# kevinh-e/BetaOne

Hardware: AMD Instinct MI355X
Metric: mcts_nodes_per_sec (higher is better)
Workload: dtype f32 (3 x f16 split, f32 accumulate)

## Files before the change

betaone_amd/csrc/bo_engine.cpp:

```cpp
#include "../../include/betaone_engine.h"
#include "../../include/betaone_lab.h"

#include "bo_tree.h"
#include "bo_fastw.h"
#include "bo_info.h"
#include "bo_select_wide.h"
#include "bo_replay.h"
#include "bo_train.h"
#include "bo_metrics.h"
#include "bo_pgn.h"
#include "bo_san.h"
#include "bo_analyse.h"
#include "bo_reanalyse.h"
#include "bo_perft.h"
#include "bo_mate.h"
#include "bo_anchor.h"
#include "bo_book.h"
#include "bo_merge.h"
#include "bo_tb.h"
#include "bo_nn_fused.h"
#include "bo_conv.h"
#include "bo_tower.h"
#include "bo_tower_wg.h"
#include "bo_tower_h.h"
#include "bo_tower_s.h"
#include "bo_tower_s16.h"
#include "bo_tower_h16.h"
#include "bo_heads.h"
#include "bo_tower_b1.h"
#include "bo_rt.h"
#include "bo_hostrng.h"

#include <math.h>
#include <stdio.h>
#include <string.h>
#include <string>
#include <vector>
#include <algorithm>
#include <deque>
#include <memory>
#include <type_traits>

static thread_local std::string g_err;
static int fail(int code, const std::string &msg) {
    g_err = msg;
    return code;
}
#define RT(call)                                                                                     \
    do {                                                                                             \
        int _rc = (call);                                                                            \
        if (_rc != 0) return fail(BO_E_HIP, std::string(#call) + ": " + rt_errstr(_rc));             \
    } while (0)

struct bo_engine {
    Eng d;
    FastW f;
    int fast_reuse = 1;
    int sel_profile = 0, sel_pending = 0;
    long long sel_launches = 0;
    double sel_ms = 0.0;
#if !defined(BO_WAVE_EMU)
// ... 482 lines not shown

static int step_launch(bo_engine *e, const float *policy_dev, const float *value_dev, int policy_kind, float *nn_in_dev, void *stream, const StepTail &vt) {
    e->prefetch_valid = false;
    if (e->fast) {
        const int rows = e->d.c.G * e->f.L;
        if (policy_kind != BO_POLICY_NONE) RT(RT_LAUNCH(bo_k_fw_apply, rows, stream, e->d, e->f, policy_dev, value_dev, policy_kind));
#if !defined(BO_WAVE_EMU)
        if (e->sel_profile) {
            if (!e->sel_ev0) { RT((int)hipEventCreate(&e->sel_ev0)); RT((int)hipEventCreate(&e->sel_ev1)); }
            if (e->sel_pending) {
                float ms = 0.0f;
                RT((int)hipEventSynchronize(e->sel_ev1));
                RT((int)hipEventElapsedTime(&ms, e->sel_ev0, e->sel_ev1));
                e->sel_ms += ms; e->sel_launches++; e->sel_pending = 0;
            }
            RT((int)hipEventRecord(e->sel_ev0, (hipStream_t)stream));
        }
#endif
        RT(launch_fw_select(e, policy_kind != BO_POLICY_NONE ? e->f.row_val : value_dev, policy_kind, stream));
#if !defined(BO_WAVE_EMU)
        if (e->sel_profile) { RT((int)hipEventRecord(e->sel_ev1, (hipStream_t)stream)); e->sel_pending = 1; }
#endif
        RT(RT_LAUNCH(bo_k_fw_leaf, rows, stream, e->d, e->f, nn_in_dev));
    } else {
        if (e->d.tb_n > 0 && (e->d.tb_flags & TBF_SEARCH)) RT(RT_LAUNCH(bo_k_step_tb, e->d.c.G, stream, e->d, policy_dev, value_dev, policy_kind, nn_in_dev, vt));
        else RT(RT_LAUNCH(bo_k_step, e->d.c.G, stream, e->d, policy_dev, value_dev, policy_kind, nn_in_dev, vt));
    }
    return BO_OK;
}
extern "C" int bo_step(bo_engine *e, const float *policy_dev, const float *value_dev, int policy_kind, float *nn_in_dev,
                       void *stream) {
    if (!e || !nn_in_dev) return fail(BO_E_ARG, "null argument");
    if (policy_kind != BO_POLICY_NONE && (!policy_dev || !value_dev)) return fail(BO_E_ARG, "policy/value required");
    return step_launch(e, policy_dev, value_dev, policy_kind, nn_in_dev, stream, StepTail{nullptr, nullptr, nullptr, nullptr, 0});
}
extern "C" int bo_step_heads(bo_engine *e, const float *logits_dev, const float *vpart_dev, const float *b1_dev, const float *w2_dev,
                             const float *b2_dev, int rows, float *nn_in_dev, void *stream) {
    if (!e || !nn_in_dev || !logits_dev || !vpart_dev || !b1_dev || !w2_dev || !b2_dev) return fail(BO_E_ARG, "null argument");
    if (e->fast) return fail(BO_E_CONFIG, "bo_step_heads: the reference-semantics search only (fast mode evaluates rows, not games)");
    if (rows < e->d.c.G) return fail(BO_E_ARG, "bo_step_heads: the partial sums must hold a row per game (rows >= G)");
    return step_launch(e, logits_dev, nullptr, BO_POLICY_LOGITS, nn_in_dev, stream, StepTail{vpart_dev, b1_dev, w2_dev, b2_dev, rows});
}

extern "C" int bo_search_poll(bo_engine *e, int32_t *n_running, int32_t *n_requested, int32_t *requested_mask, void *stream) {
    if (!e) return fail(BO_E_ARG, "null engine");
    const size_t G = (size_t)e->d.c.G;
    RT(rt_d2h(e->h_info, e->d_info_blk, 2 * G * 4, stream));
    const int *ph = e->h_info, *rq = e->h_info + G;
    RT(rt_sync(stream));
    int run = 0, req = 0;
    for (size_t g = 0; g < G; g++) {
        bool r = ph[g] == PH_RUN;
        bool q = r && rq[g] >= 0;
        run += r; req += q;
        if (requested_mask) requested_mask[g] = q ? 1 : 0;
    }
    if (n_running) *n_running = run;
    if (n_requested) *n_requested = req;
    return BO_OK;
}

extern "C" int bo_search_stop(bo_engine *e, const int32_t *stop_mask, int32_t *sims_done, void *stream) {
    if (!e) return fail(BO_E_ARG, "null engine");
    const size_t G = (size_t)e->d.c.G;
    const int *d_mask = nullptr;
    if (stop_mask) {
        memcpy(e->h_go, stop_mask, G * 4);
        RT(rt_h2d(e->d_go, e->h_go, G * 4, stream));
        d_mask = e->d_go;
    }
    if (e->fast) {
        e->prefetch_valid = false;
        RT(RT_LAUNCH(bo_k_fw_stop, e->d.c.G, stream, e->d, e->f, d_mask));
    } else {
// ... 3329 lines not shown
```

betaone_amd/csrc/bo_heads.h:

```cpp
#pragma once
#if !defined(BO_WAVE_EMU)
#include <hip/hip_runtime.h>
#include "bo_tower.h"

#define BO_HEADS_NA 4672
#define BO_HEADS_KP 128
#define BO_HEADS_KV 2048
#define BO_HEADS_NH 256
#define BO_HEADS_KS 16
#define BO_HEADS_PITCH 132

struct bo_heads_args {
    const void *p, *v;
    const float *wp, *bp, *w1, *b1, *w2, *b2;
    float *policy_out, *value_out;
    float *vpart;
    int B, softmax;
    int pb;
};
static inline int bo_heads_policy_boards(int batch) { return batch > 64 ? 128 : batch > 32 ? 64 : 32; }

struct bo_heads_pair {
    const int32_t *sel = nullptr;
    const float *wp = nullptr, *bp = nullptr, *w1 = nullptr, *b1 = nullptr, *w2 = nullptr, *b2 = nullptr;
// ... 107 lines not shown
            const int hb = 32 * (wave & 1), bb = 32 * (wave >> 1);
            bo_f32x4 acc[2][2];
#pragma unroll
            for (int c = 0; c < 2; c++)
#pragma unroll
                for (int rt = 0; rt < 2; rt++) acc[c][rt] = bo_f32x4{0, 0, 0, 0};
#pragma unroll
            for (int t = 0; t < BO_HEADS_KV / BO_HEADS_KS / 16; t++) {
                bo_f32x4 fw[2], fv[2];
#pragma unroll
                for (int c = 0; c < 2; c++) fw[c] = *reinterpret_cast<const bo_f32x4 *>(&tileW[(hb + 16 * c + i) * BO_HEADS_PITCH + 16 * t + 4 * kq]);
#pragma unroll
                for (int rt = 0; rt < 2; rt++) fv[rt] = *reinterpret_cast<const bo_f32x4 *>(&tileA[(bb + 16 * rt + i) * BO_HEADS_PITCH + 16 * t + 4 * kq]);
#pragma unroll
                for (int e = 0; e < 4; e++)
#pragma unroll
                    for (int c = 0; c < 2; c++)
#pragma unroll
                        for (int rt = 0; rt < 2; rt++) acc[c][rt] = __builtin_amdgcn_mfma_f32_16x16x4f32(fw[c][e], fv[rt][e], acc[c][rt], 0, 0, 0);
            }
#pragma unroll
            for (int c = 0; c < 2; c++)
#pragma unroll
                for (int rt = 0; rt < 2; rt++) {
                    const int row = r0 + bb + 16 * rt + i;
                    if (row < B && (only_net < 0 || (pr.sel[row] != 0) == only_net))
                        *reinterpret_cast<bo_f32x4 *>(a.vpart + ((size_t)ks * B + row) * BO_HEADS_NH + h0 + hb + 16 * c + 4 * kq) = acc[c][rt];
                }
        }
    }
}

template <bool PAIR>
__device__ __forceinline__ void bo_heads_rows_body(const bo_heads_args &a, const bo_heads_pair &q) {
    __shared__ float sred[8];
    const int tid = threadIdx.x, lane = tid & 63, wave = __builtin_amdgcn_readfirstlane(tid >> 6);
    const int B = a.B, row = (int)blockIdx.x;
    const float *b1 = a.b1, *w2 = a.w2, *b2 = a.b2;
    if constexpr (PAIR) {
        if (__builtin_amdgcn_readfirstlane(q.sel[row]) != 0) { b1 = q.b1; w2 = q.w2; b2 = q.b2; }
    }
    float part[BO_HEADS_KS];
#pragma unroll
    for (int ks = 0; ks < BO_HEADS_KS; ks++) part[ks] = a.vpart[((size_t)ks * B + row) * BO_HEADS_NH + tid];
    bo_f32x4 *r4 = reinterpret_cast<bo_f32x4 *>(a.policy_out + (size_t)row * BO_HEADS_NA);
    constexpr int N4 = BO_HEADS_NA / 4, IT = (N4 + 255) / 256;
    const float ninf = -__builtin_inff();
    bo_f32x4 x[IT];
    float mx = ninf;
    if (a.softmax) {
#pragma unroll
        for (int u = 0; u < IT; u++) {
            const int k = tid + 256 * u;
            x[u] = k < N4 ? r4[k] : bo_f32x4{ninf, ninf, ninf, ninf};
        }
    }
    float hsum = 0.0f;
#pragma unroll
    for (int ks = 0; ks < BO_HEADS_KS; ks++) hsum += part[ks];
    hsum += b1[tid];
    hsum = (hsum > 0.0f ? hsum : 0.0f) * w2[tid];
    if (a.softmax) {
#pragma unroll
        for (int u = 0; u < IT; u++) mx = fmaxf(mx, fmaxf(fmaxf(x[u][0], x[u][1]), fmaxf(x[u][2], x[u][3])));
    }
#pragma unroll
    for (int m = 32; m >= 1; m >>= 1) { mx = fmaxf(mx, __shfl_xor(mx, m, 64)); hsum += __shfl_xor(hsum, m, 64); }
    if (lane == 0) { sred[wave] = mx; sred[4 + wave] = hsum; }
    __syncthreads();
    mx = fmaxf(fmaxf(sred[0], sred[1]), fmaxf(sred[2], sred[3]));
    if (tid == 0) a.value_out[row] = tanhf(((sred[4] + sred[5]) + (sred[6] + sred[7])) + b2[0]);
    if (a.softmax) {
        float sum = 0.0f;
#pragma unroll
        for (int u = 0; u < IT; u++) {
            if (tid + 256 * u < N4) {
#pragma unroll
                for (int e = 0; e < 4; e++) { x[u][e] = expf(x[u][e] - mx); sum += x[u][e]; }
            }
        }
#pragma unroll
        for (int m = 32; m >= 1; m >>= 1) sum += __shfl_xor(sum, m, 64);
        __syncthreads();
        if (lane == 0) sred[wave] = sum;
        __syncthreads();
        sum = (sred[0] + sred[1]) + (sred[2] + sred[3]);
#pragma unroll
        for (int u = 0; u < IT; u++) {
            const int k = tid + 256 * u;
            if (k < N4) r4[k] = bo_f32x4{x[u][0] / sum, x[u][1] / sum, x[u][2] / sum, x[u][3] / sum};
        }
    }
}

extern "C" __global__ void __launch_bounds__(256)
bo_k_heads_rows(bo_heads_args a) { bo_heads_rows_body<false>(a, bo_heads_pair{}); }

extern "C" __global__ void __launch_bounds__(256)
bo_k_heads_rows_pair(bo_heads_args a, bo_heads_pair q) { bo_heads_rows_body<true>(a, q); }

typedef _Float16 bo_hh8 __attribute__((ext_vector_type(8)));

#ifndef BO_HEADS_NT_STORES
#define BO_HEADS_NT_STORES 1
// ... 224 lines not shown
```

betaone_amd/csrc/bo_tree.h:

```cpp
#pragma once
#include "bo_chess.h"
#include "bo_tb_probe.h"
#include <math.h>

#define BO_CH_CAP 32
#define BO_PATH_CAP 1024
#define BO_RES_CAP 256
#define BO_PLANES 120
#ifndef BO_PROF_SLOTS
#define BO_PROF_SLOTS 16
#endif
#define BO_ROW (BO_PLANES * 64)

enum { PH_IDLE = 0, PH_RUN = 1, PH_DONE = 2 };
enum { ST_OK = 0, ST_NODE_OVERFLOW = 1, ST_DEPTH_OVERFLOW = 2, ST_NAN_SCORE = 4, ST_PLY_OVERFLOW = 8,
       ST_ILLEGAL_ACTION = 16, ST_UL_OVERFLOW = 32, ST_TRK_OVERFLOW = 64 };
enum { POLICY_NONE = 0, POLICY_LOGITS = 1, POLICY_PROBS = 2 };

struct EngCfg {
    int G, S, B;
    int NCAP, PLY_CAP, TRK_CAP;
    int nstride;
    int UL_MAX, CH_MAX;
    float cpuct, keep;
// ... 692 lines not shown
            const float a = e.c.keep * sh.probs[idx];
            const double s2 = (double)a + e.c.eps * nz[j];
            sh.probs[idx] = (float)s2;
        }
        bo_sync();
        const float sum = np_sum_4672(sh.probs);
        const float denom = sum + 1e-12f;
        for (int j = lane; j < n; j += 64) sh.pv[j] = finite_or_zero(sh.probs[move_to_index(mv[j])] / denom, &bad);
        bo_sync();
    }
    if (bo_ballot(bad) != 0) *flags |= ST_NAN_SCORE;
    for (int j = lane; j < n; j += 64) {
        int r = stable_rank(sh.pv, n, j);
        if (r < m) sh.rank_of[BO_CH_CAP + r] = j;
    }
    bo_sync();
    for (int r = 0; r < m; r++) {
        const int j = sh.rank_of[BO_CH_CAP + r];
        bool present = false;
        for (int k = 0; k < m; k++) present = present || sh.rank_of[k] == j;
        if (!present) {
            if (lane == 0) {
                init_node(e, no, 1 + nch, 0, sh.pv[j], mv[j], make_move(P, mv[j]));
                e.root_child_rank[(size_t)g * 2 * BO_CH_CAP + nch] = j;
            }
            nch++;
        }
    }
    if (lane == 0) { e.first_child[no] = 1; e.n_children[no] = nch; e.root_nch[g] = nch; }
    *n_nodes_io = 1 + nch;
    bo_sync();
}

struct StepTail { const float *vpart, *b1, *w2, *b2; int rows; };
struct TailRegs { float part[4][16], b1[4], w2[4], b2; };
BO_DEV void tail_load(const StepTail &t, int g, TailRegs &r) {
    const int lane = bo_lane();
    BO_UNROLL
    for (int w = 0; w < 4; w++) {
        BO_UNROLL
        for (int ks = 0; ks < 16; ks++) r.part[w][ks] = t.vpart[((size_t)ks * t.rows + g) * 256 + lane + 64 * w];
        r.b1[w] = t.b1[lane + 64 * w];
        r.w2[w] = t.w2[lane + 64 * w];
    }
    r.b2 = t.b2[0];
}
BO_DEV float tail_value(const TailRegs &r) {
    float s[4];
    BO_UNROLL
    for (int w = 0; w < 4; w++) {
        float h = 0.0f;
        BO_UNROLL
        for (int ks = 0; ks < 16; ks++) h += r.part[w][ks];
        h += r.b1[w];
        s[w] = (h > 0.0f ? h : 0.0f) * r.w2[w];
    }
    for (int m = 32; m >= 1; m >>= 1) {
        BO_UNROLL
        for (int w = 0; w < 4; w++) s[w] = s[w] + bo_shfl_xor_f(s[w], m);
    }
    return tanhf(((s[0] + s[1]) + (s[2] + s[3])) + r.b2);
}

BO_DEV void apply_leaf(const Eng &e, int g, int leaf, const float *row, int kind, const float *value_of, const StepTail &vt, StepShared &sh,
                       int *n_ul_io, int *flags) {
    const size_t no = NOFF(e, g);
    const int lane = bo_lane();
    const int n = e.req_nlegal[g];
    const bo_mv *mv = e.req_moves + (size_t)g * BO_MAX_MOVES;
    int slot = *n_ul_io;
    if (slot >= e.c.UL_MAX) { *flags |= ST_UL_OVERFLOW; slot = e.c.UL_MAX - 1; }
    const size_t uo = (size_t)g * e.c.UL_MAX + slot;
    float value;
    bool bad = false;
    if (kind == POLICY_PROBS) {
        value = value_of[g];
        for (int j = lane; j < n; j += 64) sh.pv[j] = finite_or_zero(row[move_to_index(mv[j])], &bad);
    } else {
        float mx, sum;
        if (vt.vpart) {
            TailRegs tr;
            tail_load(vt, g, tr);
            row_max_sum(row, &mx, &sum);
            value = tail_value(tr);
        } else {
            value = value_of[g];
            row_max_sum(row, &mx, &sum);
        }
        for (int j = lane; j < n; j += 64) sh.pv[j] = finite_or_zero(bo_exp_row(row[move_to_index(mv[j])] - mx) / sum, &bad);
    }
    bo_sync();
    value = finite_or_zero(value, &bad);
    if (bo_ballot(bad) != 0) *flags |= ST_NAN_SCORE;
    const int M = n < e.c.CH_MAX ? n : e.c.CH_MAX;
    for (int j = lane; j < n; j += 64) {
        int r = stable_rank(sh.pv, n, j);
        if (r < M) { e.ul_move[uo * BO_CH_CAP + r] = mv[j]; e.ul_prior[uo * BO_CH_CAP + r] = sh.pv[j]; }
    }
    if (lane == 0) {
        e.ul_node[uo] = leaf;
        e.ul_nlegal[uo] = n;
        e.ul_value[uo] = value;
        e.eval_slot[no + leaf] = (short)slot;
    }
    *n_ul_io = slot + 1;
    bo_sync();
}


// ... 534 lines not shown
```

betaone_amd/engine.py:

```python
from __future__ import annotations

import ctypes as C
import os
from typing import Dict, List, Optional, Sequence, Tuple

import numpy as np
import torch

NUM_ACTIONS = 4672
INPUT_CHANNELS = 120
ROW_FLOATS = 120 * 64
MAX_LEGAL = 256
RES_CAP = 256
POLICY_NONE, POLICY_LOGITS, POLICY_PROBS = 0, 1, 2

STATUS_BITS = {1: "node overflow", 2: "depth overflow", 4: "NaN or infinite evaluation (prior or value)", 8: "ply overflow",
               16: "illegal action", 32: "leaf cache overflow", 64: "tracker overflow", 128: "position range outside the array",
               256: "pi wider than the record's rows"}
ST_PLY_OVERFLOW, ST_ILLEGAL_ACTION = 8, 16
ST_PI_OVERFLOW = 256
ST_NODE_OVERFLOW = 1
ST_DEPTH_OVERFLOW = 2
ST_NAN_SCORE = 4

# ... 46 lines not shown
                             ("pi_n", "<i4"), ("played_prob", "<f4"), ("has_old", "<i4"), ("agree", "<i4"), ("tv", "<f4"), ("phase", "<i4"),
                             ("status", "<i4"), ("ply", "<i4"), ("sims_done", "<i4"), ("watch", "<i4"), ("reserved", "<i4")])
PH_IDLE, PH_RUN, PH_DONE = 0, 1, 2
INFO_LINES, INFO_PV = 8, 24
INFO_LINE_DTYPE = np.dtype([("move", "<i4"), ("visits", "<i4"), ("w", "<f4"), ("prior", "<f4"), ("pv_len", "<i4"), ("pv", "<i4", (INFO_PV,)),
                            ("reserved", "<i4", (3,))])
INFO_DTYPE = np.dtype([("phase", "<i4"), ("status", "<i4"), ("terminal", "<i4"), ("n_legal", "<i4"), ("sims_done", "<i4"),
                       ("root_visits", "<i4"), ("arena_top", "<i4"), ("arena_granules", "<i4"), ("watch", "<i4"), ("n_lines", "<i4"),
                       ("reserved", "<i4", (6,)), ("line", INFO_LINE_DTYPE, (INFO_LINES,))])
INFO_WORDS = INFO_DTYPE.itemsize // 4


class BoHeadWeights(C.Structure):
    _fields_ = [("wp", C.c_void_p), ("bp", C.c_void_p), ("w1", C.c_void_p), ("b1", C.c_void_p), ("w2", C.c_void_p), ("b2", C.c_void_p)]


_I32P = C.POINTER(C.c_int32)
_F32P = C.POINTER(C.c_float)
_F64P = C.POINTER(C.c_double)
_TRAIN_BATCH = [C.c_int32, C.c_int32, C.c_void_p, C.c_int32, C.c_void_p, C.c_int32] + [C.c_void_p] * 3

_SYMBOLS = {
    "bo_abi_version": (C.c_int, []),
    "bo_last_error": (C.c_char_p, []),
    "bo_engine_create": (C.c_int, [C.POINTER(BoConfig), C.c_int, C.POINTER(C.c_void_p)]),
    "bo_engine_destroy": (None, [C.c_void_p]),
    "bo_games_reset": (C.c_int, [C.c_void_p, C.c_int, _I32P, C.POINTER(C.c_char_p), C.POINTER(C.c_char_p), C.c_void_p]),
    "bo_games_reset_ex": (C.c_int, [C.c_void_p, C.c_int, _I32P, C.POINTER(C.c_char_p), C.POINTER(C.c_char_p),
                                    C.POINTER(BoPosition), _I32P, C.POINTER(BoPosition), _I32P, _I32P, C.c_void_p]),
    "bo_root_info": (C.c_int, [C.c_void_p, _I32P, _I32P, _I32P, C.c_void_p]),
    "bo_search_begin": (C.c_int, [C.c_void_p, _I32P, _F64P, C.c_void_p, C.c_void_p]),
    "bo_step": (C.c_int, [C.c_void_p, C.c_void_p, C.c_void_p, C.c_int, C.c_void_p, C.c_void_p]),
    "bo_step_heads": (C.c_int, [C.c_void_p] * 6 + [C.c_int, C.c_void_p, C.c_void_p]),
    "bo_search_poll": (C.c_int, [C.c_void_p, _I32P, _I32P, _I32P, C.c_void_p]),
    "bo_search_stop": (C.c_int, [C.c_void_p, _I32P, _I32P, C.c_void_p]),
    "bo_search_close": (C.c_int, [C.c_void_p, C.c_void_p]),
    "bo_search_info": (C.c_int, [C.c_void_p, C.c_int32, C.c_void_p, C.c_void_p]),
    "bo_search_result": (C.c_int, [C.c_void_p, _I32P, _I32P, _F32P, _I32P, _I32P, _I32P, C.c_void_p]),
    "bo_play": (C.c_int, [C.c_void_p, _I32P, C.c_void_p]),
    "bo_game_export": (C.c_int, [C.c_void_p, C.c_int, C.POINTER(BoPosition), _I32P, C.c_int32, _I32P, C.c_void_p]),
    "bo_game_encode": (C.c_int, [C.c_void_p, C.c_int, C.c_int, C.c_int, C.c_void_p, C.c_void_p]),
    "bo_rng_seed": (C.c_int, [C.c_void_p, C.c_int, C.c_uint32]),
    "bo_rng_state": (C.c_int, [C.c_void_p, C.c_int, C.c_int, C.POINTER(C.c_uint32), _I32P, _I32P, _F64P]),
    "bo_selfplay_sample": (C.c_int, [C.c_void_p, _I32P, _I32P, C.c_int32, C.c_double, C.c_double, _I32P, _I32P, _F32P,
                                     _I32P, _I32P, C.c_void_p]),
    "bo_selfplay_turn": (C.c_int, [C.c_void_p, _I32P, _I32P, C.c_int32, C.c_double, C.c_double, _I32P, _I32P, _F32P, _I32P, _I32P, _I32P,
                                   C.c_void_p, _I32P, _I32P, _I32P, C.c_int32, _I32P, C.c_void_p]),
    "bo_selfplay_noise": (C.c_int, [C.c_void_p, C.c_void_p]),
    "bo_selfplay_autoturn": (C.c_int, [C.c_void_p, _I32P, _I32P, C.c_int32, C.c_double, C.c_double, _I32P, C.c_void_p, C.c_int32, C.c_void_p]),
    "bo_selfplay_autoturn_ready": (C.c_int, [C.c_void_p, _I32P]),
    "bo_selfplay_autoturn_collect": (C.c_int, [C.c_void_p, _I32P, _I32P, _F32P, _I32P, _I32P, _I32P, _I32P, _I32P, _I32P]),
    "bo_selfplay_autoturn_collect_ex": (C.c_int, [C.c_void_p, _I32P, _I32P, _F32P, _I32P, _I32P, _I32P, _I32P, _I32P, _F32P, _I32P, _I32P]),
    "bo_engine_root_values": (C.c_int, [C.c_void_p, C.c_int32]),
    "bo_selfplay_resign": (C.c_int, [C.c_void_p, _I32P, C.c_float, C.c_int32]),
    "bo_search_root_value": (C.c_int, [C.c_void_p, _F32P, C.c_void_p]),
    "bo_pgn_movetext_text": (C.c_int, [C.c_int32, C.c_void_p, C.c_void_p, C.c_int32, C.c_int32, C.c_char_p, _I32P, C.c_char_p, C.c_char_p,
                                       C.c_char_p, C.c_int64, C.POINTER(C.c_int64)]),
    "bo_search_result_prefetch": (C.c_int, [C.c_void_p, C.c_void_p]),
    "bo_selfplay_begun": (C.c_int, [C.c_void_p, _I32P, _I32P, _I32P]),
    "bo_selfplay_begin": (C.c_int, [C.c_void_p, _I32P, C.c_void_p, _I32P, _I32P, _I32P, C.c_void_p]),
    "bo_records_encode": (C.c_int, [C.c_int, C.POINTER(BoPosition), C.c_int, C.c_int, C.c_void_p, C.c_void_p]),
    "bo_fast_options": (C.c_int, [C.c_void_p, C.c_int32, C.c_int32, C.c_int32]),
    "bo_nn_tower_status": (C.c_int, [C.c_void_p, _I32P, C.c_void_p]),
    "bo_nn_tower_word": (C.c_int, [C.c_void_p, C.POINTER(C.c_void_p)]),
    "bo_replay_create": (C.c_int, [C.c_int64, C.c_int, C.c_int, C.POINTER(C.c_void_p)]),
    "bo_replay_add_game": (C.c_int, [C.c_void_p, C.c_int32, C.POINTER(BoPosition), C.c_int32, _I32P, _I32P, _F32P, _F32P, C.POINTER(C.c_int64), C.c_void_p]),
# ... 90 lines not shown
    "bo_anchor": (C.c_int, [C.c_int, C.c_int32, C.POINTER(C.c_char_p), C.c_void_p, C.c_int32, C.c_int64, C.c_uint32, C.c_void_p, C.c_void_p,
                            C.c_void_p, C.POINTER(C.c_int64), C.c_void_p]),
    "bo_anchor_eval": (C.c_int, [C.c_int, C.c_int32, C.c_void_p, C.c_void_p, C.c_void_p]),
    "bo_anchor_q": (C.c_int, [C.c_int, C.c_int32, C.POINTER(C.c_char_p), C.c_void_p, C.c_int32, C.c_int32, C.c_int64, C.c_uint32, C.c_void_p,
                              C.c_void_p, C.c_void_p, C.POINTER(C.c_int64), C.c_void_p]),
}
_LAB_SYMBOLS = {
    "bo_debug_tree": (C.c_int, [C.c_void_p, C.c_int, C.POINTER(BoNode), C.c_int32, _I32P, C.c_void_p]),
    "bo_debug_search_state": (C.c_int, [C.c_void_p, _I32P, C.c_void_p]),
    "bo_debug_fast": (C.c_int, [C.c_void_p, C.c_int, _I32P, C.c_int32, _I32P, C.c_void_p]),
    "bo_event_pair_overhead": (C.c_int, [_F64P, C.c_int32, C.c_void_p]),
    "bo_nn_b1_profile": (C.c_int, [C.c_void_p, C.c_int, C.POINTER(C.c_uint64), C.c_int]),
    "bo_fast_stats": (C.c_int, [C.c_void_p, C.POINTER(C.c_uint64), C.POINTER(C.c_uint64), _I32P, C.c_int32, _F64P, C.POINTER(C.c_int64),
                               C.c_void_p]),
    "bo_debug_profile": (C.c_int, [C.c_void_p, C.c_int, C.POINTER(C.c_uint64), C.c_void_p]),
    "bo_debug_stamp": (C.c_int, [C.c_void_p, C.c_uint64, C.c_uint64, C.c_void_p]),
    "bo_nn_tower_forward_timed": (C.c_int, [C.c_void_p, C.c_void_p, C.c_void_p, C.c_void_p, C.c_void_p, C.c_int, C.c_void_p, C.c_void_p]),
    "bo_select_wide": (C.c_int, [C.c_void_p, C.c_void_p, C.c_void_p, C.c_void_p, C.c_int, C.c_int, C.c_float, C.c_int,
                                 C.c_void_p, C.c_void_p, C.c_void_p]),
}

HIP_LIB_PATH = os.path.join(os.path.dirname(os.path.abspath(__file__)), "csrc", "libbetaone_hip.so")


def bind(cdll: C.CDLL) -> C.CDLL:
    for name, (res, args) in list(_SYMBOLS.items()) + list(_LAB_SYMBOLS.items()):
        fn = getattr(cdll, name)
        fn.restype = res
        fn.argtypes = args
    return cdll


_hip_lib: Optional[C.CDLL] = None
ABI_VERSION = 22
PROF_SLOTS = 16
METRIC_ROW = {name: k for k, name in enumerate((
    "BAD", "HAS_POLICY", "DECISIVE", "RANK", "TOP1", "TOP3", "TOP5", "ARGMAX_IN_SUPPORT", "CE", "TARGET_ENTROPY", "NET_ENTROPY", "P_TOP",
    "P_SUPPORT", "SE_Z", "SE_Q", "ABS_V", "SIGN_OK", "Z", "V"))}
METRIC = {name: k for k, name in enumerate((
    "N_ROWS", "N_BAD", "N_POLICY_ROWS", "N_DECISIVE", "SUM_RANK", "SUM_TOP1", "SUM_TOP3", "SUM_TOP5", "SUM_ARGMAX_IN_SUPPORT", "SUM_CE",
    "SUM_TARGET_ENTROPY", "SUM_NET_ENTROPY", "SUM_P_TOP", "SUM_P_SUPPORT", "SUM_SE_Z", "SUM_SE_Q", "SUM_ABS_V", "SUM_SIGN_OK", "SUM_Z", "SUM_V"))}
METRIC_ROW_COLS, METRIC_COLS = len(METRIC_ROW), len(METRIC)


def load_hip_library() -> C.CDLL:
    global _hip_lib
    if _hip_lib is None:
        from . import build as _build

        if not os.path.exists(HIP_LIB_PATH):
            raise EngineError(f"{HIP_LIB_PATH} is missing: build it with `python -m betaone_amd.build` "
                              "(hipcc --offload-arch=gfx950); betaone_amd has no CPU fallback")
        if _build.needs_build():
            raise EngineError(f"{HIP_LIB_PATH} was not built from the sources next to it (csrc/*.h changed since): "
                              "run `python -m betaone_amd.build`")
        _hip_lib = bind(C.CDLL(HIP_LIB_PATH))
        if _hip_lib.bo_abi_version() != ABI_VERSION:
            raise EngineError(f"libbetaone_hip.so ABI version {_hip_lib.bo_abi_version()} != {ABI_VERSION} (include/betaone_engine.h)")
    return _hip_lib


def runtime_device(requested) -> torch.device:
    dev = torch.device(requested)
    if dev.type != "cuda":
        raise EngineError(f"betaone_amd runs on an MI355X (device 'cuda' / 'cuda:N', got {requested!r}); there is no CPU path")
    return torch.device("cuda", dev.index if dev.index is not None else torch.cuda.current_device())

# ... 137 lines not shown

    def search_begin_dev(self, want_ptr: int, nn_in_ptr: int, stream: int = 0):
        self._check(self.lib.bo_search_begin_dev(self.h, want_ptr, nn_in_ptr, stream))

    def analysis_result(self, played_ptr: int, out_ptr: int, stream: int = 0):
        self._check(self.lib.bo_analysis_result(self.h, played_ptr or None, out_ptr, stream))

    def reanalysis_result(self, played_action_ptr: int, root_ptr: int, old_ptr_ptr: int, old_idx_ptr: int, old_val_ptr: int, W: int,
                          out_ptr: int, pi_idx_ptr: int, pi_val_ptr: int, stream: int = 0):
        self._check(self.lib.bo_reanalysis_result(self.h, played_action_ptr or None, root_ptr or None, old_ptr_ptr or None, old_idx_ptr or None,
                                                  old_val_ptr or None, int(W), out_ptr, pi_idx_ptr, pi_val_ptr, stream))

    def root_info(self, stream: int = 0):
        nl, tm, ply = (np.zeros(self.G, dtype=np.int32) for _ in range(3))
        self._check(self.lib.bo_root_info(self.h, _p(nl), _p(tm), _p(ply), stream))
        return nl, tm, ply

    def match_select(self, net_of_white_ptr: int, sel_ptr: int, stream: int = 0):
        self._check(self.lib.bo_match_select(self.h, net_of_white_ptr, sel_ptr, stream))

    def search_begin(self, go, noise: Optional[np.ndarray], nn_in_ptr: int, stream: int = 0):
        g = _i32(go)
        nz = None
        if noise is not None:
            nz = np.ascontiguousarray(noise, dtype=np.float64).reshape(self.G, MAX_LEGAL)
        self._check(self.lib.bo_search_begin(self.h, _p(g), _p(nz, _F64P) if nz is not None else None, nn_in_ptr, stream))

    def step(self, policy_ptr: int, value_ptr: int, kind: int, nn_in_ptr: int, stream: int = 0):
        self._check(self.lib.bo_step(self.h, policy_ptr, value_ptr, kind, nn_in_ptr, stream))

    def step_heads(self, logits_ptr: int, vpart_ptr: int, b1_ptr: int, w2_ptr: int, b2_ptr: int, rows: int, nn_in_ptr: int, stream: int = 0):
        self._check(self.lib.bo_step_heads(self.h, logits_ptr, vpart_ptr, b1_ptr, w2_ptr, b2_ptr, rows, nn_in_ptr, stream))

    def poll(self, stream: int = 0, want_mask: bool = True):
        run, req = C.c_int32(), C.c_int32()
        mask = np.zeros(self.G, dtype=np.int32) if want_mask else None
        self._check(self.lib.bo_search_poll(self.h, C.byref(run), C.byref(req), _p(mask) if want_mask else None, stream))
        return run.value, req.value, mask

    def search_stop(self, mask=None, stream: int = 0) -> np.ndarray:
        m = _i32(mask) if mask is not None else None
        done = np.zeros(self.G, dtype=np.int32)
        self._check(self.lib.bo_search_stop(self.h, _p(m) if m is not None else None, _p(done), stream))
        return done

    def search_info(self, n_lines: int, out_ptr: int, stream: int = 0) -> None:
        self._check(self.lib.bo_search_info(self.h, int(n_lines), out_ptr, stream))

    def search_close(self, stream: int = 0) -> None:
        self._check(self.lib.bo_search_close(self.h, stream))

    def result(self, stream: int = 0) -> Dict[str, np.ndarray]:
        G = self.G
        out = dict(n=np.zeros(G, np.int32), idx=np.zeros((G, RES_CAP), np.int32), val=np.zeros((G, RES_CAP), np.float32),
                   best_idx=np.zeros(G, np.int32), best_move=np.zeros(G, np.int32), total=np.zeros(G, np.int32))
        self._check(self.lib.bo_search_result(self.h, _p(out["n"]), _p(out["idx"]), _p(out["val"], _F32P),
                                              _p(out["best_idx"]), _p(out["best_move"]), _p(out["total"]), stream))
        return out

    def play(self, actions, stream: int = 0):
        a = _i32(actions)
        assert a.shape == (self.G,)
        self._check(self.lib.bo_play(self.h, _p(a), stream))

    def rng_seed(self, slot: int, seed: int):
        self._check(self.lib.bo_rng_seed(self.h, slot, seed & 0xFFFFFFFF))
# ... 215 lines not shown
```

betaone_amd/rollout.py:

```python
from __future__ import annotations

import math
import os
import time
from dataclasses import dataclass, field
from typing import Callable, Dict, List, Optional, Sequence

import numpy as np
import torch

from . import engine as E
from . import sampling

CAPTURE_MODE = "thread_local"


@dataclass
class GameState:
    game_id: int
    rng: object
    start_fen: Optional[str] = None
    start_fullmove: int = 1
    start_white: bool = True
    plies: int = 0
# ... 176 lines not shown
        self.device_turn = os.environ.get("BETAONE_DEVICE_TURN", "1") != "0"
        self._begun_want = None
        self._active = np.zeros(G, dtype=bool)
        self._plies = np.zeros(G, dtype=np.int64)
        self._start_full = np.ones(G, dtype=np.int64)
        self._start_black = np.zeros(G, dtype=np.int64)
        self._start_step = np.zeros(G, dtype=np.int64)
        self._first_ply = np.zeros(G, dtype=np.int64)
        self._step = 0
        self._hist = {}
        self._pk = 0 if self.fast else 2
        self._pi_n = np.zeros((G, 256), np.int32)
        self._pi_idx = np.zeros((G, 256, max(1, self._pk)), np.int32)
        self._pi_val = np.zeros((G, 256, max(1, self._pk)), np.float32)
        self._out = dict(n=np.zeros(G, np.int32), idx=np.zeros((G, E.RES_CAP), np.int32), val=np.zeros((G, E.RES_CAP), np.float32),
                         best_idx=np.zeros(G, np.int32), action=np.zeros(G, np.int32))
        if self.values:
            self._out.update(root_value=np.zeros(G, np.float32), resigned=np.zeros(G, np.int32))
        self._rv = np.zeros((G, 256 if self.values else 0), np.float32)
        self._resigned = np.zeros(G, dtype=bool)
        self._renable = np.zeros(G, dtype=np.int32)
        self._rcheck = np.zeros(G, dtype=bool)
        self._rcnt = np.zeros((G, 2), dtype=np.int64)
        self.net_of_white = torch.zeros(G, dtype=torch.int32, device=self.device) if self.pair else None
        self._sel = torch.zeros(G, dtype=torch.int32, device=self.device) if self.pair else None
        self._watch_net()
        self._set_tail()

    def _set_tail(self):
        m = self.model
        ok = (self.policy_kind == E.POLICY_LOGITS and not self.fast and not self.autocast and self.device.type == "cuda"
              and os.environ.get("BETAONE_STEP_TAIL", "1") != "0" and hasattr(m, "forward_tail") and m.tail_supported(self.G))
        self.step_tail = bool(ok)
        self._tail_params = tuple(m.tail_params()) if ok else None

    def _step_after(self, first, second):
        if self.step_tail:
            if second.shape != (16, self.G, 256):
                raise E.EngineError(f"step tail: value_fc1's partial sums must be [16, {self.G}, 256], got {tuple(second.shape)}")
            self.eng.step_heads(first.data_ptr(), second.data_ptr(), *self._tail_params, second.shape[1], self.nn_in.data_ptr(), self._stream())
        else:
            self.eng.step(first.data_ptr(), second.data_ptr(), self.policy_kind, self.nn_in.data_ptr(), self._stream())

    def _watch_net(self):
        inner = getattr(self.model, "net", self.model)
        words = getattr(inner, "overflow_words", None)
        self._watch_msg = getattr(inner, "OVERFLOW_MESSAGE", "the evaluate stage reported a fault")
        ptr, n = words() if words is not None else (0, 1)
        self.eng.watch(ptr, n)

    def _check_watch(self):
        if self.eng.watch_seen():
            chk = getattr(getattr(self.model, "net", self.model), "check_overflow", None)
            if chk is not None and self.device.type == "cuda":
                torch.cuda.synchronize(self.device)
                chk()
            raise E.EngineError(self._watch_msg)

    def _stream(self) -> int:
        return torch.cuda.current_stream(self.device).cuda_stream if self.device.type == "cuda" else 0

    def _forward(self):
        if self.tower_timing is not None:
            getattr(self.model, "net", self.model).tower_timing_buf = self.tower_timing
        want_probs = self.policy_kind == E.POLICY_PROBS
        if self.pair:
            self.eng.match_select(self.net_of_white.data_ptr(), self._sel.data_ptr(), self._stream())
            logits, value = (self.model.forward_probs if want_probs else self.model)(self.nn_in, self._sel)
            return logits.float().contiguous(), value.float().contiguous()
        fused = getattr(self.model, "forward_probs", None) if (want_probs and not self.autocast) else None
        with torch.no_grad():
            if self.step_tail:
                logits, part = self.model.forward_tail(self.nn_in)
                return logits, part
            if fused is not None:
                logits, value = fused(self.nn_in)
                want_probs = False
            elif self.autocast:
                with torch.autocast(self.device.type):
                    logits, value = self.model(self.nn_in)
            else:
                logits, value = self.model(self.nn_in)
        logits = logits.float()
        if want_probs:
            logits = torch.softmax(logits, dim=1)
        return logits.contiguous(), value.float().contiguous()

    def _eval_and_step_eager(self):
        self._stamp(1)
        logits, value = self._forward()
        self._stamp(2)
        self._logits, self._value = logits, value
        self._step_after(logits, value)
        self._stamp(3)

    def _capture(self):
        side = torch.cuda.Stream(self.device)
        side.wait_stream(torch.cuda.current_stream(self.device))
        with torch.cuda.stream(side):
            for _ in range(2):
                self._forward()
        torch.cuda.current_stream(self.device).wait_stream(side)
        torch.cuda.synchronize(self.device)
        g = torch.cuda.CUDAGraph()
        with torch.cuda.graph(g, capture_error_mode=CAPTURE_MODE):
            logits, value = self._forward()
            self._step_after(logits, value)
        self._graph, self._logits, self._value = g, logits, value

    def _eval_and_step(self):
        self.n_forward += 1
        if self.use_graph:
            if self._graph is None:
                self._capture()
            self._graph.replay()
        else:
            self._eval_and_step_eager()

    MAX_GRAPH_ITERATIONS = 12

    def _eval_and_step_n(self, n: int, close: Optional[bool] = None):
        if close is None:
            close = self.close_last_eval
        close = bool(close) and n >= 2
        iters = n - 1 if close else n
        if n <= 1 or not self.use_graph:
            for _ in range(iters):
                self._eval_and_step()
            if close:
                self.eng.search_close(self._stream())
            return
        if n > self.MAX_GRAPH_ITERATIONS:
            while n > 0:
                k = min(n, self.MAX_GRAPH_ITERATIONS)
                self._eval_and_step_n(k, close and k == n)
                n -= k
            return
        key = (n, True) if close else n
        g = self._graphs_n.get(key)
        if g is None:
            if self._graph is None:
# ... 145 lines not shown
        th, ti, tf = self.temperature
        for g in np.nonzero(live)[0]:
            gs = self.games[g]
            if mask[g]:
                actions[g] = int(ext[g])
                gs.pis.append((np.zeros(0, np.int32), np.zeros(0, np.float32)))
            else:
                n = int(res["n"][g])
                idx, val = res["idx"][g, :n].copy(), res["val"][g, :n].copy()
                actions[g] = sampling.select_action_sparse(idx, val, gs.fullmove_number(), gs.rng, th, ti, tf)
                gs.pis.append((idx, val))
            gs.plies += 1
        self.host_seconds += time.perf_counter() - t0
        self.eng.play(actions, self._stream())
        if while_searching is not None:
            while_searching()
        n_moves = int(np.count_nonzero(live))
        self.n_plies += n_moves
        return n_moves

    def _resign_decide(self, go, rv, plies) -> np.ndarray:
        out = np.zeros(self.G, dtype=bool)
        if not self.resign:
            return out
        for g in np.nonzero(np.asarray(go, bool) & (self._renable != 0))[0]:
            par = int(plies[g]) & 1
            c = self._rcnt[g, par] + 1 if np.float32(rv[g]) < self.resign_t else 0
            self._rcnt[g, par] = c
            out[g] = c >= self.resign_k
        return out

    def _forward_only(self):
        if not self.use_graph:
            self._f_logits, self._f_value = self._forward()
            return
        if self._fgraph is None:
            if self._graph is None:
                self._capture()
            g = torch.cuda.CUDAGraph()
            with torch.cuda.graph(g, capture_error_mode=CAPTURE_MODE):
                logits, value = self._forward()
            self._fgraph, self._f_logits, self._f_value = g, logits, value
        self._fgraph.replay()

    PLY_TRACE = []

    def _pp(self, name):
        now = time.perf_counter()
        self.ply_profile.append((name, now - self._pp_t))
        if os.environ.get("BO_PLY_PROFILE") == "trace":
            Rollout.PLY_TRACE.append((self._pp_t, now, self._stamp_id, name))
        self._pp_t = now

    def _run_search_steps(self, poll: bool = True):
        burst = self.expected_evals
        info = None
        if self._noise_pending:
            self._noise_pending = False
            if self._fwd_early:
                self._fwd_early = False
            else:
                self.n_forward += 1
                self._forward_only()
            if self._begun is E.LAZY_BEGIN:
                info = self.eng.selfplay_begun()
                self._begun = None
            if self.ply_profile is not None: self._pp("begun")
            self.eng.selfplay_noise(self._stream())
            if self.ply_profile is not None: self._pp("noise")
            self._step_after(self._f_logits, self._f_value)
            burst -= 1
        while True:
            self._eval_and_step_n(burst)
            if not poll:
# ... 522 lines not shown
```

include/betaone_engine.h:

```cpp
#ifndef BETAONE_ENGINE_H
#define BETAONE_ENGINE_H

#include <stdint.h>

#ifdef __cplusplus
extern "C" {
#endif

#define BO_ABI_VERSION 22
#define BO_NUM_ACTIONS 4672
#define BO_INPUT_CHANNELS 120
#define BO_ROW_FLOATS (120 * 64)
#define BO_MAX_LEGAL 256
#define BO_RES_CAP 256

enum {
    BO_OK = 0,
    BO_E_ARG = -1,
    BO_E_HIP = -2,
    BO_E_CONFIG = -3,
    BO_E_FEN = -4,
    BO_E_STATE = -5
};

enum {
    BO_ST_NODE_OVERFLOW = 1, BO_ST_DEPTH_OVERFLOW = 2, BO_ST_NAN_SCORE = 4, BO_ST_PLY_OVERFLOW = 8,
    BO_ST_ILLEGAL_ACTION = 16, BO_ST_UL_OVERFLOW = 32, BO_ST_TRK_OVERFLOW = 64,
    BO_ST_BAD_RANGE = 128,
    BO_ST_PI_OVERFLOW = 256
};

enum { BO_POLICY_NONE = 0, BO_POLICY_LOGITS = 1, BO_POLICY_PROBS = 2 };

typedef struct {
    int32_t n_games;
    int32_t num_simulations;
    int32_t mcts_batch_size;
    int32_t max_plies;
    double cpuct;
    double widen_coeff;
    double dirichlet_alpha;
    double dirichlet_epsilon;
// ... 5 lines not shown
typedef struct {
    uint64_t bb[8];
    int32_t turn;
    uint32_t castling;
    int32_t ep_square;
    int32_t ep_key;
    int32_t halfmove_clock;
    int32_t fullmove_number;
} bo_position;

typedef struct bo_engine bo_engine;

int bo_abi_version(void);
const char *bo_last_error(void);

int bo_engine_create(const bo_config *cfg, int device, bo_engine **out);
void bo_engine_destroy(bo_engine *e);

int bo_games_reset(bo_engine *e, int n, const int32_t *slots, const char *const *fens, const char *const *moves,
                   void *stream);

int bo_games_reset_ex(bo_engine *e, int n, const int32_t *slots, const char *const *fens, const char *const *moves,
                      const bo_position *hist, const int32_t *n_hist, const bo_position *trk,
                      const int32_t *trk_counts, const int32_t *trk_off, void *stream);

int bo_root_info(bo_engine *e, int32_t *n_legal, int32_t *terminal, int32_t *ply, void *stream);

int bo_search_begin(bo_engine *e, const int32_t *go, const double *noise, float *nn_in_dev, void *stream);

int bo_step(bo_engine *e, const float *policy_dev, const float *value_dev, int policy_kind, float *nn_in_dev,
            void *stream);
int bo_step_heads(bo_engine *e, const float *logits_dev, const float *vpart_dev, const float *b1_dev, const float *w2_dev,
                  const float *b2_dev, int rows, float *nn_in_dev, void *stream);

int bo_search_poll(bo_engine *e, int32_t *n_running, int32_t *n_requested, int32_t *requested_mask, void *stream);

int bo_search_stop(bo_engine *e, const int32_t *stop_mask, int32_t *sims_done, void *stream);

int bo_search_close(bo_engine *e, void *stream);

int bo_search_result(bo_engine *e, int32_t *res_n, int32_t *res_idx, float *res_val, int32_t *best_idx,
                     int32_t *best_move, int32_t *total_visits, void *stream);

int bo_play(bo_engine *e, const int32_t *action, void *stream);

int bo_rng_seed(bo_engine *e, int slot, uint32_t seed);
int bo_rng_state(bo_engine *e, int slot, int set, uint32_t *key624, int32_t *pos, int32_t *has_gauss, double *gauss);
int bo_selfplay_sample(bo_engine *e, const int32_t *active, const int32_t *move_number, int32_t threshold,
                       double t_initial, double t_final, int32_t *res_n, int32_t *res_idx, float *res_val,
                       int32_t *best_idx, int32_t *action_out, void *stream);
int bo_selfplay_begin(bo_engine *e, const int32_t *want, float *nn_in_dev, int32_t *n_legal_out, int32_t *terminal_out,
                      int32_t *go_out, void *stream);

int bo_selfplay_turn(bo_engine *e, const int32_t *active, const int32_t *move_number, int32_t threshold, double t_initial,
                     double t_final, int32_t *res_n, int32_t *res_idx, float *res_val, int32_t *best_idx, int32_t *action_out,
                     const int32_t *want_next, float *nn_in_dev, int32_t *n_legal_out, int32_t *terminal_out, int32_t *go_out,
                     int32_t defer_noise, int32_t *completed, void *stream);
int bo_selfplay_begun(bo_engine *e, int32_t *n_legal_out, int32_t *terminal_out, int32_t *go_out);
int bo_search_result_prefetch(bo_engine *e, void *stream);
int bo_selfplay_noise(bo_engine *e, void *stream);

int bo_selfplay_autoturn(bo_engine *e, const int32_t *active, const int32_t *move_number, int32_t threshold, double t_initial,
                         double t_final, const int32_t *want_next, float *nn_in_dev, int32_t redo, void *stream);
int bo_selfplay_autoturn_ready(bo_engine *e, int32_t *ready_out);
int bo_selfplay_autoturn_collect(bo_engine *e, int32_t *res_n, int32_t *res_idx, float *res_val, int32_t *best_idx, int32_t *action_out,
                                 int32_t *n_legal_out, int32_t *terminal_out, int32_t *go_out, int32_t *completed);
// ... 346 lines not shown
```

Measured before the change: 80.74 million.

## Fuse heads row softmax/value kernel with MCTS step for probability policy

Adds a bo_rows_step kernel that, per game, computes the value-head tail and the in-place policy softmax, then runs the MCTS step body in the same workgroup with the value passed through shared memory. In probability-policy mode the rollout now uses forward_tail and this fused kernel instead of a separate heads kernel followed by a step kernel. This removes a kernel launch and a global round trip between them. The cost is that the step work now runs on a single wave inside a 256-thread block, and the rows kernel's occupancy and structure become coupled to the step's.

```diff
diff --git a/betaone_amd/csrc/bo_engine.cpp b/betaone_amd/csrc/bo_engine.cpp
--- a/betaone_amd/csrc/bo_engine.cpp
+++ b/betaone_amd/csrc/bo_engine.cpp
@@ -27,6 +27,7 @@
 #include "bo_tower_s16.h"
 #include "bo_tower_h16.h"
 #include "bo_heads.h"
+#include "bo_rows_step.h"
 #include "bo_tower_b1.h"
 #include "bo_rt.h"
 #include "bo_hostrng.h"
@@ -575,14 +576,36 @@
                        void *stream) {
     if (!e || !nn_in_dev) return fail(BO_E_ARG, "null argument");
     if (policy_kind != BO_POLICY_NONE && (!policy_dev || !value_dev)) return fail(BO_E_ARG, "policy/value required");
-    return step_launch(e, policy_dev, value_dev, policy_kind, nn_in_dev, stream, StepTail{nullptr, nullptr, nullptr, nullptr, 0});
+    return step_launch(e, policy_dev, value_dev, policy_kind, nn_in_dev, stream, StepTail{nullptr, nullptr, nullptr, nullptr, 0, nullptr});
 }
 extern "C" int bo_step_heads(bo_engine *e, const float *logits_dev, const float *vpart_dev, const float *b1_dev, const float *w2_dev,
                              const float *b2_dev, int rows, float *nn_in_dev, void *stream) {
     if (!e || !nn_in_dev || !logits_dev || !vpart_dev || !b1_dev || !w2_dev || !b2_dev) return fail(BO_E_ARG, "null argument");
     if (e->fast) return fail(BO_E_CONFIG, "bo_step_heads: the reference-semantics search only (fast mode evaluates rows, not games)");
     if (rows < e->d.c.G) return fail(BO_E_ARG, "bo_step_heads: the partial sums must hold a row per game (rows >= G)");
-    return step_launch(e, logits_dev, nullptr, BO_POLICY_LOGITS, nn_in_dev, stream, StepTail{vpart_dev, b1_dev, w2_dev, b2_dev, rows});
+    return step_launch(e, logits_dev, nullptr, BO_POLICY_LOGITS, nn_in_dev, stream, StepTail{vpart_dev, b1_dev, w2_dev, b2_dev, rows, nullptr});
+}
+extern "C" int bo_rows_step(bo_engine *e, float *logits_inout_dev, const float *vpart_dev, const float *b1_dev, const float *w2_dev,
+                            const float *b2_dev, float *value_out_dev, int rows, float *nn_in_dev, void *stream) {
+    if (!e || !nn_in_dev || !logits_inout_dev || !vpart_dev || !b1_dev || !w2_dev || !b2_dev || !value_out_dev) return fail(BO_E_ARG, "null argument");
+    if (e->fast) return fail(BO_E_CONFIG, "bo_rows_step: the reference-semantics search only (fast mode evaluates rows, not games)");
+    if (rows < e->d.c.G) return fail(BO_E_ARG, "bo_rows_step: the partial sums must hold a row per game (rows >= G)");
+#if defined(BO_WAVE_EMU)
+    (void)stream;
+    return fail(BO_E_CONFIG, "bo_rows_step is a gfx950-only kernel");
+#else
+    e->prefetch_valid = false;
+    bo_heads_args a;
+    a.p = a.v = nullptr; a.wp = a.bp = a.w1 = nullptr;
+    a.b1 = b1_dev; a.w2 = w2_dev; a.b2 = b2_dev;
+    a.policy_out = logits_inout_dev; a.value_out = value_out_dev; a.vpart = const_cast<float *>(vpart_dev);
+    a.B = rows; a.softmax = 1; a.pb = bo_heads_policy_boards(rows);
+    const unsigned G = (unsigned)e->d.c.G;
+    if (e->d.tb_n > 0 && (e->d.tb_flags & TBF_SEARCH)) hipLaunchKernelGGL(bo_k_rows_step_tb, dim3(G), dim3(256), 0, (hipStream_t)stream, e->d, a, nn_in_dev);
+    else hipLaunchKernelGGL(bo_k_rows_step, dim3(G), dim3(256), 0, (hipStream_t)stream, e->d, a, nn_in_dev);
+    RT((int)hipGetLastError());
+    return BO_OK;
+#endif
 }
 
 extern "C" int bo_search_poll(bo_engine *e, int32_t *n_running, int32_t *n_requested, int32_t *requested_mask, void *stream) {
diff --git a/betaone_amd/csrc/bo_heads.h b/betaone_amd/csrc/bo_heads.h
--- a/betaone_amd/csrc/bo_heads.h
+++ b/betaone_amd/csrc/bo_heads.h
@@ -163,7 +163,7 @@
 }
 
 template <bool PAIR>
-__device__ __forceinline__ void bo_heads_rows_body(const bo_heads_args &a, const bo_heads_pair &q) {
+__device__ __forceinline__ void bo_heads_rows_body(const bo_heads_args &a, const bo_heads_pair &q, float *value_keep = nullptr) {
     __shared__ float sred[8];
     const int tid = threadIdx.x, lane = tid & 63, wave = __builtin_amdgcn_readfirstlane(tid >> 6);
     const int B = a.B, row = (int)blockIdx.x;
@@ -200,7 +200,11 @@
     if (lane == 0) { sred[wave] = mx; sred[4 + wave] = hsum; }
     __syncthreads();
     mx = fmaxf(fmaxf(sred[0], sred[1]), fmaxf(sred[2], sred[3]));
-    if (tid == 0) a.value_out[row] = tanhf(((sred[4] + sred[5]) + (sred[6] + sred[7])) + b2[0]);
+    if (tid == 0) {
+        const float value = tanhf(((sred[4] + sred[5]) + (sred[6] + sred[7])) + b2[0]);
+        a.value_out[row] = value;
+        if (value_keep) *value_keep = value;
+    }
     if (a.softmax) {
         float sum = 0.0f;
 #pragma unroll
diff --git a/betaone_amd/csrc/bo_rows_step.h b/betaone_amd/csrc/bo_rows_step.h
--- /dev/null
+++ b/betaone_amd/csrc/bo_rows_step.h
@@ -0,0 +1,25 @@
+#pragma once
+#if !defined(BO_WAVE_EMU)
+#include <hip/hip_runtime.h>
+#include "bo_heads.h"
+#include "bo_tree.h"
+
+template <bool TB>
+__device__ __forceinline__ void bo_rows_step_body(const Eng &e, const bo_heads_args &a, float *nn_in) {
+    __shared__ StepShared sh;
+    __shared__ float value_here;
+    const int g = (int)blockIdx.x;
+    bo_heads_rows_body<false>(a, bo_heads_pair{}, &value_here);
+    __builtin_amdgcn_fence(__ATOMIC_RELEASE, "workgroup");
+    __syncthreads();
+    if (__builtin_amdgcn_readfirstlane((int)threadIdx.x >> 6) != 0) return;
+    if (e.phase[g] != PH_RUN) return;
+    step_body<TB>(e, g, a.policy_out, a.value_out, POLICY_PROBS, nn_in, sh, StepTail{nullptr, nullptr, nullptr, nullptr, 0, &value_here});
+}
+
+extern "C" __global__ void __launch_bounds__(256)
+bo_k_rows_step(Eng e, bo_heads_args a, float *nn_in) { bo_rows_step_body<false>(e, a, nn_in); }
+
+extern "C" __global__ void __launch_bounds__(256)
+bo_k_rows_step_tb(Eng e, bo_heads_args a, float *nn_in) { bo_rows_step_body<true>(e, a, nn_in); }
+#endif
diff --git a/betaone_amd/csrc/bo_tree.h b/betaone_amd/csrc/bo_tree.h
--- a/betaone_amd/csrc/bo_tree.h
+++ b/betaone_amd/csrc/bo_tree.h
@@ -748,7 +748,7 @@
     bo_sync();
 }
 
-struct StepTail { const float *vpart, *b1, *w2, *b2; int rows; };
+struct StepTail { const float *vpart, *b1, *w2, *b2; int rows; const float *value_here; };
 struct TailRegs { float part[4][16], b1[4], w2[4], b2; };
 BO_DEV void tail_load(const StepTail &t, int g, TailRegs &r) {
     const int lane = bo_lane();
@@ -790,7 +790,7 @@
     float value;
     bool bad = false;
     if (kind == POLICY_PROBS) {
-        value = value_of[g];
+        value = vt.value_here ? *vt.value_here : value_of[g];
         for (int j = lane; j < n; j += 64) sh.pv[j] = finite_or_zero(row[move_to_index(mv[j])], &bad);
     } else {
         float mx, sum;
diff --git a/betaone_amd/engine.py b/betaone_amd/engine.py
--- a/betaone_amd/engine.py
+++ b/betaone_amd/engine.py
@@ -102,6 +102,7 @@
     "bo_search_begin": (C.c_int, [C.c_void_p, _I32P, _F64P, C.c_void_p, C.c_void_p]),
     "bo_step": (C.c_int, [C.c_void_p, C.c_void_p, C.c_void_p, C.c_int, C.c_void_p, C.c_void_p]),
     "bo_step_heads": (C.c_int, [C.c_void_p] * 6 + [C.c_int, C.c_void_p, C.c_void_p]),
+    "bo_rows_step": (C.c_int, [C.c_void_p] * 7 + [C.c_int, C.c_void_p, C.c_void_p]),
     "bo_search_poll": (C.c_int, [C.c_void_p, _I32P, _I32P, _I32P, C.c_void_p]),
     "bo_search_stop": (C.c_int, [C.c_void_p, _I32P, _I32P, C.c_void_p]),
     "bo_search_close": (C.c_int, [C.c_void_p, C.c_void_p]),
@@ -258,7 +259,7 @@
 
 
 _hip_lib: Optional[C.CDLL] = None
-ABI_VERSION = 22
+ABI_VERSION = 23
 PROF_SLOTS = 16
 METRIC_ROW = {name: k for k, name in enumerate((
     "BAD", "HAS_POLICY", "DECISIVE", "RANK", "TOP1", "TOP3", "TOP5", "ARGMAX_IN_SUPPORT", "CE", "TARGET_ENTROPY", "NET_ENTROPY", "P_TOP",
@@ -462,6 +463,10 @@
     def step_heads(self, logits_ptr: int, vpart_ptr: int, b1_ptr: int, w2_ptr: int, b2_ptr: int, rows: int, nn_in_ptr: int, stream: int = 0):
         self._check(self.lib.bo_step_heads(self.h, logits_ptr, vpart_ptr, b1_ptr, w2_ptr, b2_ptr, rows, nn_in_ptr, stream))
 
+    def rows_step(self, logits_ptr: int, vpart_ptr: int, b1_ptr: int, w2_ptr: int, b2_ptr: int, value_ptr: int, rows: int, nn_in_ptr: int,
+                  stream: int = 0):
+        self._check(self.lib.bo_rows_step(self.h, logits_ptr, vpart_ptr, b1_ptr, w2_ptr, b2_ptr, value_ptr, rows, nn_in_ptr, stream))
+
     def poll(self, stream: int = 0, want_mask: bool = True):
         run, req = C.c_int32(), C.c_int32()
         mask = np.zeros(self.G, dtype=np.int32) if want_mask else None
diff --git a/betaone_amd/rollout.py b/betaone_amd/rollout.py
--- a/betaone_amd/rollout.py
+++ b/betaone_amd/rollout.py
@@ -232,10 +232,19 @@
         ok = (self.policy_kind == E.POLICY_LOGITS and not self.fast and not self.autocast and self.device.type == "cuda"
               and os.environ.get("BETAONE_STEP_TAIL", "1") != "0" and hasattr(m, "forward_tail") and m.tail_supported(self.G))
         self.step_tail = bool(ok)
-        self._tail_params = tuple(m.tail_params()) if ok else None
+        rs = (self.policy_kind == E.POLICY_PROBS and not self.fast and not self.autocast and not self.pair and self.device.type == "cuda"
+              and os.environ.get("BETAONE_ROWS_STEP", "1") != "0" and hasattr(m, "forward_tail") and m.tail_supported(self.G))
+        self.rows_step = bool(rs)
+        self._tail_params = tuple(m.tail_params()) if ok or rs else None
+        self._rs_value = torch.empty((self.G, 1), dtype=torch.float32, device=self.device) if rs else None
 
     def _step_after(self, first, second):
-        if self.step_tail:
+        if self.rows_step and second.dim() == 3:
+            if second.shape != (16, self.G, 256):
+                raise E.EngineError(f"rows step: value_fc1's partial sums must be [16, {self.G}, 256], got {tuple(second.shape)}")
+            self.eng.rows_step(first.data_ptr(), second.data_ptr(), *self._tail_params, self._rs_value.data_ptr(), second.shape[1],
+                               self.nn_in.data_ptr(), self._stream())
+        elif self.step_tail:
             if second.shape != (16, self.G, 256):
                 raise E.EngineError(f"step tail: value_fc1's partial sums must be [16, {self.G}, 256], got {tuple(second.shape)}")
             self.eng.step_heads(first.data_ptr(), second.data_ptr(), *self._tail_params, second.shape[1], self.nn_in.data_ptr(), self._stream())
@@ -260,7 +269,7 @@
     def _stream(self) -> int:
         return torch.cuda.current_stream(self.device).cuda_stream if self.device.type == "cuda" else 0
 
-    def _forward(self):
+    def _forward(self, step_follows: bool = True):
         if self.tower_timing is not None:
             getattr(self.model, "net", self.model).tower_timing_buf = self.tower_timing
         want_probs = self.policy_kind == E.POLICY_PROBS
@@ -270,7 +279,7 @@
             return logits.float().contiguous(), value.float().contiguous()
         fused = getattr(self.model, "forward_probs", None) if (want_probs and not self.autocast) else None
         with torch.no_grad():
-            if self.step_tail:
+            if self.step_tail or (self.rows_step and step_follows):
                 logits, part = self.model.forward_tail(self.nn_in)
                 return logits, part
             if fused is not None:
@@ -292,6 +301,8 @@
         self._stamp(2)
         self._logits, self._value = logits, value
         self._step_after(logits, value)
+        if self.rows_step:
+            self._part, self._value = value, self._rs_value
         self._stamp(3)
 
     def _capture(self):
@@ -307,6 +318,8 @@
             logits, value = self._forward()
             self._step_after(logits, value)
         self._graph, self._logits, self._value = g, logits, value
+        if self.rows_step:
+            self._part, self._value = value, self._rs_value
 
     def _eval_and_step(self):
         self.n_forward += 1
@@ -518,14 +531,14 @@
 
     def _forward_only(self):
         if not self.use_graph:
-            self._f_logits, self._f_value = self._forward()
+            self._f_logits, self._f_value = self._forward(step_follows=False)
             return
         if self._fgraph is None:
             if self._graph is None:
                 self._capture()
             g = torch.cuda.CUDAGraph()
             with torch.cuda.graph(g, capture_error_mode=CAPTURE_MODE):
-                logits, value = self._forward()
+                logits, value = self._forward(step_follows=False)
             self._fgraph, self._f_logits, self._f_value = g, logits, value
         self._fgraph.replay()
 
diff --git a/include/betaone_engine.h b/include/betaone_engine.h
--- a/include/betaone_engine.h
+++ b/include/betaone_engine.h
@@ -7,7 +7,7 @@
 extern "C" {
 #endif
 
-#define BO_ABI_VERSION 22
+#define BO_ABI_VERSION 23
 #define BO_NUM_ACTIONS 4672
 #define BO_INPUT_CHANNELS 120
 #define BO_ROW_FLOATS (120 * 64)
@@ -79,6 +79,8 @@
             void *stream);
 int bo_step_heads(bo_engine *e, const float *logits_dev, const float *vpart_dev, const float *b1_dev, const float *w2_dev,
                   const float *b2_dev, int rows, float *nn_in_dev, void *stream);
+int bo_rows_step(bo_engine *e, float *logits_inout_dev, const float *vpart_dev, const float *b1_dev, const float *w2_dev,
+                 const float *b2_dev, float *value_out_dev, int rows, float *nn_in_dev, void *stream);
 
 int bo_search_poll(bo_engine *e, int32_t *n_running, int32_t *n_requested, int32_t *requested_mask, void *stream);
 
```

Result: no change. 81.44 million (median of 6 runs) (+0.9%).
